# wenz116/lang2seg

Hardware: AMD Instinct MI355X
Metric: train images/sec (cycle loss on), 600×1000 input, at 1/2/4/8 MI355X (higher is better)
Workload: dtype bf16; 1 GPU; train_cycle.sh step: ResNet-101 C4 + 7 spatial dynamic filters + att2in2 cycle loss, 600x1000 image, 20-token expression (V=3349), 12000->2000 proposals, 256 RoIs, per-GPU batch 1; variant=cycle, parallelism=dp1

## Files before the change

include/lang2seg_hip.h:

```cpp
#ifndef LANG2SEG_HIP_H
#define LANG2SEG_HIP_H
#include <stdint.h>
#ifdef __HIPCC__
#include <hip/hip_runtime.h>
#else
typedef struct ihipStream_t* hipStream_t;
#endif
#ifdef __cplusplus
extern "C" {
#endif

#define L2S_F32 0
#define L2S_BF16 1

int l2s_version(void);

#define L2S_CONV_RELU 1
#define L2S_CONV_OUT_F32 4
#define L2S_CONV_DECONV2X2 8
#define L2S_CONV_SCATTER 16
#define L2S_ALGO_AUTO 0
#define L2S_ALGO_STAGED 1
#define L2S_ALGO_DMA 2
#define L2S_ALGO_DMA_STAMPED 4
// ... 5 lines not shown
#define L2S_ALGO_DMA256 9
#define L2S_ALGO_WS64_STAMPED 8
typedef struct {
  const void* x;
  const void* w;
  void* y;
  const float* bias;
  const void* add;
  const void* ref;
  int n_img, IH, IW, Cin, OH, OW, Cout, KH, KW, stride, pad;
  int ldx, ldy, ldadd, ldref;
  int flags;
  int out_h, out_w, out_stride;
  int tile;
  int split_k;
  int xcd_mode;
  int algo;
  float* ws;
  size_t ws_floats;
  int prio;
} l2s_conv_desc;
int l2s_conv_igemm(const l2s_conv_desc* d, int dtype, hipStream_t stream);
const char* l2s_conv_plan_name(const l2s_conv_desc* d, int dtype);
const char* l2s_last_kernel(void);

typedef struct {
  const void* dy;
  const void* x;
  float* dw;
  int n_img, IH, IW, Cin, OH, OW, Cout, KH, KW, stride, pad;
  int lddy, ldx;
  int split_k;
  int tile;
  float* ws;
  size_t ws_bytes;
} l2s_wgrad_desc;
size_t l2s_wgrad_ws_bytes(const l2s_wgrad_desc* d, int dtype);

#define L2S_WGRAD_MAX_GROUP 64
#define L2S_WGRAD_MAX_SEG 2
typedef struct {
  const void* dy[L2S_WGRAD_MAX_SEG];
  const void* x[L2S_WGRAD_MAX_SEG];
  int n_img[L2S_WGRAD_MAX_SEG], IH[L2S_WGRAD_MAX_SEG], IW[L2S_WGRAD_MAX_SEG], OH[L2S_WGRAD_MAX_SEG], OW[L2S_WGRAD_MAX_SEG];
  int lddy[L2S_WGRAD_MAX_SEG], ldx[L2S_WGRAD_MAX_SEG];
  float* dw;
// ... 370 lines not shown
```

lang2seg_amd/_lib.py:

```python
import ctypes as C
import os

_HERE = os.path.dirname(os.path.abspath(__file__))
LIB_PATH = os.path.join(_HERE, 'lib', 'liblang2seg_hip.so')
F32, BF16 = 0, 1

vp, i32, i64, f32, u64, sz = C.c_void_p, C.c_int, C.c_long, C.c_float, C.c_uint64, C.c_size_t


class ConvDesc(C.Structure):
    _fields_ = [('x', vp), ('w', vp), ('y', vp), ('bias', vp), ('add', vp), ('ref', vp),
                ('n_img', i32), ('IH', i32), ('IW', i32), ('Cin', i32), ('OH', i32), ('OW', i32), ('Cout', i32),
                ('KH', i32), ('KW', i32), ('stride', i32), ('pad', i32),
                ('ldx', i32), ('ldy', i32), ('ldadd', i32), ('ldref', i32), ('flags', i32),
                ('out_h', i32), ('out_w', i32), ('out_stride', i32), ('tile', i32), ('split_k', i32), ('xcd_mode', i32), ('algo', i32), ('ws', vp), ('ws_floats', sz), ('prio', i32)]


class RoiBlock0Desc(C.Structure):
    _fields_ = [('feat', vp), ('rois', vp), ('w1', vp), ('b1', vp), ('w2', vp), ('b2', vp), ('pooled', vp), ('y1', vp), ('y2', vp),
                ('H', i32), ('W', i32), ('C', i32), ('R', i32), ('P', i32), ('N1', i32), ('N2', i32), ('spatial_scale', C.c_float), ('debug', i32)]


class WgradDesc(C.Structure):
    _fields_ = [('dy', vp), ('x', vp), ('dw', vp),
# ... 84 lines not shown


class BeamStepArgs(C.Structure):
    _fields_ = [('logits', vp), ('ld_logits', i32)] + [(n, i32) for n in ('V1', 'B', 't', 'T', 'R', 'n_state')] + \
               [(n, vp) for n in ('beam_seq', 'beam_seq_logprobs', 'beam_logprobs_sum')] + \
               [('state_in', vp * 4), ('state_out', vp * 4), ('ld_in', i32 * 4), ('ld_out', i32 * 4)] + \
               [(n, vp) for n in ('next_tokens', 'parents', 'done', 'done_count')]


class SgdSeg(C.Structure):
    _fields_ = [('offset', i64), ('count', i64), ('row_len', i32), ('weight_decay', i32), ('rowscale_off', i64),
                ('lr_mult', f32), ('chunk0', i32), ('flags', i32), ('reserved', i32)]


CONV_RELU, CONV_OUT_F32, CONV_DECONV2X2, CONV_SCATTER = 1, 4, 8, 16
LOSS_RPN_CLS, LOSS_RPN_BOX, LOSS_CLS, LOSS_BOX, LOSS_MASK, LOSS_CAP, LOSS_TOTAL, LOSS_RESPONSE = range(8)

SIGS = {
    'l2s_version': (i32, []),
    'l2s_conv_plan_name': (C.c_char_p, [vp, i32]),
    'l2s_last_kernel': (C.c_char_p, []),
    'l2s_roialign_block0_fwd': (i32, [C.POINTER(RoiBlock0Desc), vp]),
    'l2s_conv_igemm': (i32, [C.POINTER(ConvDesc), i32, vp]),
    'l2s_conv_wgrad': (i32, [C.POINTER(WgradDesc), i32, vp]),
    'l2s_wgrad_ws_bytes': (sz, [C.POINTER(WgradDesc), i32]),
    'l2s_wgrad_variant': (i32, [i32, i32, i32, i32, i32, i32, i32, i64, i32]),
    'l2s_wgrad_tiles': (i64, [i32, i32, i32, i32, i32]),
    'l2s_conv_wgrad_grouped': (i32, [vp, vp, i32, i32, i32, vp, sz, vp]),
    'l2s_weight_cast': (i32, [vp, vp, vp, i32, i32, i32, i32, vp]),
    'l2s_weight_transpose': (i32, [vp, vp, vp, i32, i32, i32, i32, vp]),
    'l2s_colsum': (i32, [vp, i32, i32, i32, vp, vp, i64, i32, vp]),
    'l2s_weight_transpose_batched': (i32, [vp, i32, i32, i32, vp]),
    'l2s_stem_conv': (i32, [vp, vp, vp, vp, vp, i32, i32, i32, i32, i32, vp]),
    'l2s_stem_pack_bytes': (C.c_size_t, []),
    'l2s_stem_pack': (i32, [vp, vp, vp]),
    'l2s_stem_pool_bf16': (i32, [vp, vp, vp, vp, vp, i32, i32, i32, i32, i32, i32, vp]),
    'l2s_maxpool3x3s2': (i32, [vp, vp, i32, i32, i32, i32, i32, i32, vp]),
    'l2s_fill_f32': (i32, [vp, f32, i64, vp]),
    'l2s_cast': (i32, [vp, i32, vp, i32, i64, vp]),
    'l2s_add3': (i32, [vp, vp, vp, vp, i64, i32, vp]),
    'l2s_avgpool_fwd': (i32, [vp, vp, i32, i32, i32, i32, vp]),
    'l2s_avgpool_bwd': (i32, [vp, vp, vp, vp, i32, i32, i32, i32, vp]),
    'l2s_adaptive_pool_fwd': (i32, [vp, vp, vp, i32, i32, i32, i32, i32, i32, i32, vp]),
    'l2s_adaptive_pool_bwd': (i32, [vp, i32, i32, i32, vp, vp, vp, i32, i32, i32, i32, i32, i32, vp]),
    'l2s_mask_downsample': (i32, [vp, vp, i32, i32, i32, i32, vp]),
    'l2s_dropout_mask': (i32, [vp, i64, f32, vp, u64, vp]),
# ... 187 lines not shown
```

lang2seg_amd/csrc/conv_igemm.hip:

```cpp
#include "common.h"
#include "roi_sample.h"
#include "../../include/lang2seg_hip.h"
#include <stdlib.h>
#include <type_traits>

namespace {

template <typename T> struct Mma;
template <> struct Mma<bf16_t> {
  static __device__ __forceinline__ f32x4 run(const uint4& a, const uint4& b, f32x4 c) {
    return __builtin_amdgcn_mfma_f32_16x16x32_bf16(__builtin_bit_cast(bf16x8, a), __builtin_bit_cast(bf16x8, b), c, 0, 0, 0);
  }
};
template <> struct Mma<float> {
  static __device__ __forceinline__ f32x4 run(const uint4& a, const uint4& b, f32x4 c) {
    c = __builtin_amdgcn_mfma_f32_16x16x4f32(__uint_as_float(a.x), __uint_as_float(b.x), c, 0, 0, 0);
    c = __builtin_amdgcn_mfma_f32_16x16x4f32(__uint_as_float(a.y), __uint_as_float(b.y), c, 0, 0, 0);
    c = __builtin_amdgcn_mfma_f32_16x16x4f32(__uint_as_float(a.z), __uint_as_float(b.z), c, 0, 0, 0);
    c = __builtin_amdgcn_mfma_f32_16x16x4f32(__uint_as_float(a.w), __uint_as_float(b.w), c, 0, 0, 0);
    return c;
  }
};

constexpr int ROWB = 128;
// ... 1405 lines not shown
  const int rrow = lane >> 4, rch = lane & 15;
#pragma unroll
  for (int i = 0; i < TM; ++i) {
    if (i + 1 < TM) fetch(i + 1, ov[(i + 1) & 1]);
#pragma unroll
    for (int j = 0; j < TN; ++j) {
      const u32x2 oo = ov[i & 1][j];
      float v[4] = {acc[i][j][0] + bv[j][0], acc[i][j][1] + bv[j][1], acc[i][j][2] + bv[j][2], acc[i][j][3] + bv[j][3]};
      if constexpr (BOTH) igemm_finish<4, false>(p, v, oo, rv[i & 1][j]);
      else igemm_finish<4, false>(p, v, oo, oo);
      *(u32x2*)(wlds + fr * 256 + (((2 * j + (fg >> 1)) ^ fr) << 4) + ((fg & 1) << 3)) = igemm_pack_bf<u32x2>(v);
    }
#pragma unroll
    for (int h = 0; h < 4; ++h) {
      const int row = rrow + 4 * h;
      const u32x4v q = *(const u32x4v*)(wlds + row * 256 + ((rch ^ row) << 4));
      const int m = m0 + wm * WM + i * 16 + row, n = n0 + wn * WN + rch * 8;
      const unsigned o = (m < M && n < p.Cout) ? (unsigned)(((long)m * p.ldy + n) * 2) : NOPE;
      __builtin_amdgcn_raw_buffer_store_b128(q, ry, o, 0, 0);
    }
  }
}

__global__ __launch_bounds__(512) void igemm_dma256_kernel(const l2s_conv_desc p) {
  typedef bf16_t T;
  constexpr int BM = 256, BN = 256, WM = 64, WN = 128, TM = 4, TN = 8;
  constexpr int RB = 64;
  constexpr int STG = (BM + BN) * RB;
  constexpr int NP = 4;
  extern __shared__ __attribute__((aligned(16))) char smem[];
  const int tid = threadIdx.x, lane = tid & 63;
  const int wave = __builtin_amdgcn_readfirstlane(tid >> 6);
  const int grp = wave >> 2;
  const int wm = wave >> 1, wn = wave & 1;
  const int M = p.n_img * p.OH * p.OW;
  const int K = p.Cin;
  int mt, nt;
  igemm_tile_of(blockIdx.x, (M + BM - 1) / BM, (p.Cout + BN - 1) / BN, p.xcd_mode, mt, nt);
  const int m0 = mt * BM, n0 = nt * BN;
  const unsigned lds0 = (unsigned)(uintptr_t)(__attribute__((address_space(3))) char*)smem;
  i32x4s rx, rw;
  rx.x = (int)(uintptr_t)p.x; rx.y = (int)((uintptr_t)p.x >> 32); rx.z = (int)(((long)(M - 1) * p.ldx + p.Cin) * 2L); rx.w = 0x00020000;
  rw.x = (int)(uintptr_t)p.w; rw.y = (int)((uintptr_t)p.w >> 32); rw.z = (int)((long)p.Cout * K * 2L); rw.w = 0x00020000;
  const int prow = lane >> 2, sch = (lane & 3) ^ ((prow >> 2) & 3);
  unsigned voA[2], voB[2];
#pragma unroll
  for (int j = 0; j < 2; ++j) {
    const int m = m0 + 16 * (wave + 8 * j) + prow, n = n0 + 16 * (wave + 8 * j) + prow;
    voA[j] = m < M ? (unsigned)(((long)m * p.ldx + sch * 8) * 2L) : OOR;
    voB[j] = n < p.Cout ? (unsigned)(((long)n * K + sch * 8) * 2L) : OOR;
  }
  const int KT = K / 32;
  const unsigned ldsA = lds0 + (unsigned)(wave * 1024), ldsB = ldsA + (unsigned)(BM * RB);
  auto request = [&](int stage, int t) {
    const unsigned sb = (unsigned)(stage * STG), so = (unsigned)(t * RB);
#pragma unroll
    for (int j = 0; j < 2; ++j) dma_b128(rx, voA[j], so, ldsA + sb + (unsigned)(j * 8192));
#pragma unroll
    for (int j = 0; j < 2; ++j) dma_b128(rw, voB[j], so, ldsB + sb + (unsigned)(j * 8192));
  };
  f32x4 acc[TM][TN];
#pragma unroll
  for (int i = 0; i < TM; ++i)
#pragma unroll
    for (int j = 0; j < TN; ++j) acc[i][j] = (f32x4){0.f, 0.f, 0.f, 0.f};
  const int fr = lane & 15, fg = lane >> 4;
  const int ch = (fg ^ ((fr >> 2) & 3)) << 4;
  const int offa = (wm * WM + fr) * RB + ch, offb = BM * RB + (wn * WN + fr) * RB + ch;
  uint4 fa[TM], fb[TN];
  auto read_all = [&](int stage) {
    const char* base = smem + stage * STG;
#pragma unroll
    for (int i = 0; i < TM; ++i) fa[i] = *(const uint4*)(base + offa + i * 16 * RB);
#pragma unroll
    for (int j = 0; j < TN; ++j) fb[j] = *(const uint4*)(base + offb + j * 16 * RB);
  };
  auto mma_all = [&]() {
#pragma unroll
    for (int i = 0; i < TM; ++i)
#pragma unroll
      for (int j = 0; j < TN; ++j) acc[i][j] = Mma<T>::run(fb[j], fa[i], acc[i][j]);
  };
// ... 6 lines not shown
  for (int t = 0; t < KT; ++t) {
    const int st2 = st == 0 ? 2 : st - 1;
    read_all(st);
    if (t + 2 < KT) request(st2, t + 2);
    wait_lgkm0();
    if (grp == 1) {
      if (t + 2 < KT) asm volatile("s_waitcnt vmcnt(%0)" ::"n"(NP) : "memory");
      else asm volatile("s_waitcnt vmcnt(0)" ::: "memory");
    }
    wg_barrier();
    __builtin_amdgcn_sched_barrier(0);
    mma_all();
    __builtin_amdgcn_sched_barrier(0);
    if (grp == 0) {
      if (t + 2 < KT) asm volatile("s_waitcnt vmcnt(%0)" ::"n"(NP) : "memory");
      else asm volatile("s_waitcnt vmcnt(0)" ::: "memory");
    }
    wg_barrier();
    st = st == 2 ? 0 : st + 1;
  }
  if (grp == 0) wg_barrier();
  if (p.add && p.ref) igemm_epilogue_wave128<TM, TN, true>(p, acc, m0, n0, wm, wn, lane, M, smem + 3 * STG + wave * 4096);
  else igemm_epilogue_wave128<TM, TN, false>(p, acc, m0, n0, wm, wn, lane, M, smem + 3 * STG + wave * 4096);
}

template <int BM, int BN>
__global__ __launch_bounds__(512) void igemm_pdma_kernel(const l2s_conv_desc p) {
  typedef bf16_t T;
  constexpr int WGM = 4, WGN = 2, WM = BM / WGM, WN = BN / WGN, TM = WM / 16, TN = WN / 16;
  constexpr int PA = BM / 64, PB = BN / 64, NP = PA + PB;
  constexpr int STG = (BM + BN) * ROWB;
  extern __shared__ __attribute__((aligned(16))) char smem[];
  const int tid = threadIdx.x, lane = tid & 63;
  const int wave = __builtin_amdgcn_readfirstlane(tid >> 6);
  const int grp = wave >> 2;
  const int wm = wave >> 1, wn = wave & 1;
  const int M = p.n_img * p.OH * p.OW;
  const int K = p.Cin;
  const int KT = K / 64;
  const int MT = (M + BM - 1) / BM, NT = (p.Cout + BN - 1) / BN, G = MT * NT;
  const int ntl = (G - (int)blockIdx.x + (int)gridDim.x - 1) / (int)gridDim.x;
  auto tile_of = [&](int i, int& m0_, int& n0_) {
    int mt, nt;
    igemm_tile_of(blockIdx.x + i * gridDim.x, MT, NT, p.xcd_mode, mt, nt);
    m0_ = mt * BM; n0_ = nt * BN;
  };
// ... 622 lines not shown
int launch_igemm_p3(const l2s_conv_desc& d, hipStream_t st) {
  const int M = d.n_img * d.OH * d.OW;
  const size_t lds = (size_t)NS * 4 * ((PR / 16 + 9 * BN / 16 + 3) / 4) * 1024;
  IGEMM_LAUNCH_RETURN((igemm_p3_kernel<BN, PR, NS>), dim3(cdiv(M, 128) * cdiv(d.Cout, BN)), dim3(512), lds, st, d);
}

template <int BM, int BN, bool STAMP = false>
int launch_igemm_dma(const l2s_conv_desc& d, hipStream_t st) {
  const int M = d.n_img * d.OH * d.OW;
  const size_t lds = (size_t)3 * (BM + BN) * ROWB + (STAMP ? 8192 : 0);
  IGEMM_LAUNCH_RETURN((igemm_dma_kernel<BM, BN, STAMP>), dim3(cdiv(M, BM) * cdiv(d.Cout, BN)), dim3(512), lds, st, d);
}

int launch_igemm_dma196(const l2s_conv_desc& d, hipStream_t st) {
  const int M = d.n_img * d.OH * d.OW;
  const size_t lds = (size_t)3 * (256 + 128) * ROWB;
  IGEMM_LAUNCH_RETURN(igemm_dma196_kernel, dim3(cdiv(M, T196) * cdiv(d.Cout, 128)), dim3(512), lds, st, d);
}

int launch_igemm_dma256(const l2s_conv_desc& d, hipStream_t st) {
  const int M = d.n_img * d.OH * d.OW;
  const size_t lds = (size_t)3 * 512 * 64 + 8 * 4096;
  IGEMM_LAUNCH_RETURN(igemm_dma256_kernel, dim3(cdiv(M, 256) * cdiv(d.Cout, 256)), dim3(512), lds, st, d);
}

template <int BM, int BN>
int launch_igemm_pdma(const l2s_conv_desc& d, hipStream_t st) {
  const int M = d.n_img * d.OH * d.OW;
  const int G = cdiv(M, BM) * cdiv(d.Cout, BN);
  const int cap = l2s_knobs::pdma_wgs > 0 ? (l2s_knobs::pdma_wgs & ~7) : 256;
  const int grid = G < cap ? ((G + 7) & ~7) : cap;
  const size_t lds = (size_t)3 * (BM + BN) * ROWB + 8 * 2048;
  IGEMM_LAUNCH_RETURN((igemm_pdma_kernel<BM, BN>), dim3(grid), dim3(512), lds, st, d);
}
#undef IGEMM_LAUNCH_RETURN
#undef IGEMM_LAUNCH

}


enum ConvPlan { PLAN_EINVAL = 0, PLAN_GENERIC64, PLAN_GENERIC128, PLAN_RING64, PLAN_RING128, PLAN_WS64, PLAN_KS64, PLAN_KS64_D3, PLAN_SP224, PLAN_SP256,
                PLAN_DMA256, PLAN_DMA256_STAMPED, PLAN_WS64_SPLITK, PLAN_P3_32_256, PLAN_P3_64_256, PLAN_P3_32_384, PLAN_P3_64_384, PLAN_RING128X64, PLAN_PDMA256, PLAN_DMA256X256, PLAN_DMA196 };
static const char* const PLAN_NAMES[] = {"invalid", "igemm_kernel<64,64>", "igemm_kernel<128,128>", "igemm_ring_kernel<64,64>", "igemm_ring_kernel<128,128>",
                                         "igemm_ws64_kernel", "igemm_ks64_kernel<4>", "igemm_ks64_kernel<3>", "igemm_sp_kernel<224,128>", "igemm_sp_kernel<256,128>",
                                         "igemm_dma_kernel<256,128>", "igemm_dma_kernel<256,128,stamped>", "igemm_ws64_kernel + splitk_reduce_kernel", "igemm_p3_kernel<32,256>", "igemm_p3_kernel<64,256>", "igemm_p3_kernel<32,384>", "igemm_p3_kernel<64,384>", "igemm_ring_kernel<128,64>", "igemm_pdma_kernel<256,128>", "igemm_dma256_kernel", "igemm_dma196_kernel"};
static ConvPlan conv_plan(const l2s_conv_desc* d, int dtype, bool* tapin_out) {
// ... 89 lines not shown
    case PLAN_P3_64_256: return launch_igemm_p3<64, 256, 3>(dd, stream);
    case PLAN_P3_32_384: return launch_igemm_p3<32, 384, 3>(dd, stream);
    case PLAN_P3_64_384: return launch_igemm_p3<64, 384, 2>(dd, stream);
    case PLAN_KS64: return launch_igemm_ks64<4>(dd, stream);
    case PLAN_KS64_D3: return launch_igemm_ks64<3>(dd, stream);
    case PLAN_WS64:
      if (d->algo == L2S_ALGO_WS64_STAMPED) return launch_igemm_ws64<3, 64, true>(dd, stream);
      return launch_igemm_ws64<3, 64>(dd, stream);
    case PLAN_WS64_SPLITK: return launch_igemm_ws64<3, 64>(dd, stream, splitk_factor(dd, d->KH * d->KW * d->Cin / 64));
    case PLAN_SP224: return BYT(OUT_TAP(launch_igemm_sp, bf16_t, 224, 128, 2, 4, 2), OUT_TAP(launch_igemm_sp, float, 224, 128, 2, 4, 2));
    case PLAN_SP256: return BYT(OUT_TAP(launch_igemm_sp, bf16_t, 256, 128, 4, 2, 2), OUT_TAP(launch_igemm_sp, float, 256, 128, 4, 2, 2));
    case PLAN_RING128X64: return launch_igemm_ring<bf16_t, 128, 64, 2, 2, 2, false>(dd, stream);
    case PLAN_RING128: return BYT(OUT(launch_igemm_ring, bf16_t, 128, 128, 2, 2, 2), OUT(launch_igemm_ring, float, 128, 128, 2, 2, 2));
    case PLAN_RING64: return BYT(OUT(launch_igemm_ring, bf16_t, 64, 64, 2, 2, 2), OUT(launch_igemm_ring, float, 64, 64, 2, 2, 4));
    case PLAN_GENERIC128: return BYT(OUT(launch_igemm, bf16_t, 128, 128), OUT(launch_igemm, float, 128, 128));
    case PLAN_GENERIC64: return BYT(OUT(launch_igemm, bf16_t, 64, 64), OUT(launch_igemm, float, 64, 64));
    default: return L2S_EINVAL;
  }
#undef BYT
#undef OUT
#undef OUT_TAP
}

extern "C" int l2s_roialign_block0_fwd(const l2s_roi_block0_desc* d, hipStream_t stream) {
  if (!d || !d->feat || !d->rois || !d->w1 || !d->w2 || !d->pooled || !d->y1 || !d->y2) return L2S_EINVAL;
  const int PP = d->P * d->P;
  if (d->R <= 0 || PP < 1 || PP > 64 || d->C % 128 || d->N1 % 128 || d->N2 % 128 || d->N1 <= 0 || d->N2 <= 0) return L2S_EINVAL;
  if ((size_t)PP * d->C * 2 + 64 * sizeof(RoiTaps) > 160 * 1024) return L2S_EINVAL;
  if ((long)d->H * d->W * d->C * 2 >= (1L << 31) || (long)d->N1 * d->C * 2 >= (1L << 31) || (long)d->N2 * d->C * 2 >= (1L << 31)) return L2S_EINVAL;
  return launch_roialign_block0(*d, stream);
}
```

lang2seg_amd/nets/network.py:

```python
import numpy as np
import os
import torch

from .. import ops as O
from .._lib import F32, BF16, LOSS_CAP
from ..model.config import cfg
from .params import ParamStore
from . import anchors as ANC


class ConvOp(object):

    def __init__(self, net, wkey, Cin, Cout, k=1, stride=1, pad=0, bias_key=None, need_dgrad=True, group=None, Cout_pad=None, full_map=False):
        self.net, self.wkey, self.Cin, self.Cout, self.k, self.stride, self.pad = net, wkey, Cin, Cout, k, stride, pad
        self.full_map = bool(full_map and k > 1 and pad == 0 and stride == 1)
        self.t_taps, self.t_cin = (1, k * k * Cin) if self.full_map else (k * k, Cin)
        self.bias_key, self.need_dgrad, self.group = bias_key, need_dgrad, group
        self.Np = Cout if Cout_pad is None else Cout_pad
        self.prio = 1 if str(wkey).startswith(('resnet.layer1.', 'resnet.layer2.', 'resnet.layer3.')) and getattr(net, 'chain_prio', True) else 0
        P = net.P
        taps = k * k
        cnt = self.Np * taps * Cin
        if group is not None:
            self.trainable = True
# ... 11 lines not shown
            else:
                self.w_master = P.frozen[wkey].view(-1)
                self.w_grad = None
                self.wf = O.empty((cnt,), net.dt)
            if bias_key is not None and bias_key in P.offsets:
                self.bias = P.view(bias_key); self.bias_grad = P.view(bias_key, P.grad)
            elif bias_key is not None:
                self.bias = P.frozen[bias_key]; self.bias_grad = None
            else:
                self.bias = P.bn_bias.get(wkey); self.bias_grad = None
        self.wb = O.empty((cnt,), net.dt) if (need_dgrad and self.trainable) else None
        net.convs.append(self)

    def refresh(self, full=False):
        taps = self.k * self.k
        if not self.trainable and full:
            O.weight_cast(self.w_master, self.scale, self.wf, self.Np, taps, self.Cin)
        if self.wb is not None:
            O.weight_transpose(self.w_master, self.scale, self.wb, self.Np, self.t_taps, self.t_cin)

    def out_hw(self, IH, IW):
        return (IH + 2 * self.pad - self.k) // self.stride + 1, (IW + 2 * self.pad - self.k) // self.stride + 1

    def fwd(self, x, n, IH, IW, y, add=None, relu=False, out_f32=False, tile=0):
        OH, OW = self.out_hw(IH, IW)
        O.conv_igemm(x, self.wf, y, n, IH, IW, self.Cin, OH, OW, self.Np, self.k, self.k, self.stride, self.pad,
                     bias=self.bias, add=add, relu=relu, out_f32=out_f32, tile=tile, dt=self.net.dt, ws=self.net.splitk_ws(n * OH * OW * self.Np), prio=max(self.prio, self.net.prio_floor),
                     algo=(self.net.conv_algo if self.k == 1 and self.stride == 1 and self.Np >= 1024 else None))
        return y

    def dgrad(self, g, n, IH, IW, dx, add=None, ref=None):
        OH, OW = self.out_hw(IH, IW)
        if self.full_map:
            assert IH == self.k and IW == self.k and OH == 1 and OW == 1
            O.conv_igemm(g, self.wb, dx, n, 1, 1, self.Np, 1, 1, self.t_cin, 1, 1, 1, 0, add=add, ref=ref, dt=self.net.dt,
                         prio=max(self.prio, self.net.prio_floor))
            return dx
        if self.stride == 1:
            O.conv_igemm(g, self.wb, dx, n, OH, OW, self.Np, IH, IW, self.Cin, self.k, self.k, 1, self.k - 1 - self.pad,
                         add=add, ref=ref, dt=self.net.dt, ws=self.net.splitk_ws(n * IH * IW * self.Cin), prio=max(self.prio, self.net.prio_floor),
                         algo=(self.net.conv_algo if self.k == 1 and self.Cin >= 1024 else None))
        else:
            assert self.k == 1
            O.conv_igemm(g, self.wb, dx, n, OH, OW, self.Np, OH, OW, self.Cin, 1, 1, 1, 0, add=add, ref=ref,
                         scatter=(IH, IW, self.stride), dt=self.net.dt, prio=max(self.prio, self.net.prio_floor))
        return dx

    def wgrad(self, g, x, n, IH, IW):
        ko = self.net.knockout
        if 'wgrad' in ko or ('wgrad4' in ko and str(self.wkey).startswith('resnet.layer4.')) or \
                ('wgrad3' in ko and str(self.wkey).startswith(('resnet.layer3.', 'resnet.layer2.'))):
            return
        OH, OW = self.out_hw(IH, IW)
        self.net.wgq.add(self.w_grad, g, x, n, IH, IW, self.Cin, OH, OW, self.Np, self.k, self.stride, self.pad)
# ... 104 lines not shown
                        ctx.__enter__()
                    O.call('l2s_conv_wgrad_grouped', ent[1].data_ptr(), C.cast(arr, C.c_void_p), len(chunk), v, dt, ws.data_ptr(),
                           ws.numel() * 4, O.stream())
                    if ctx is not None:
                        ctx.__exit__(None, None, None)
        return True

    V5_STREAM = 'wg'
    SMALL_M_TILE = 0
    MIN_WG = 256
    V4_FILL = 128


class Bottleneck(object):

    def __init__(self, net, prefix, inplanes, planes, stride, has_down, need_dx=True):
        self.net, self.prefix, self.stride, self.need_dx = net, prefix, stride, need_dx
        self.inpl, self.planes = inplanes, planes
        self.c1 = ConvOp(net, prefix + '.conv1.weight', inplanes, planes, 1, stride, 0, need_dgrad=need_dx)
        self.c2 = ConvOp(net, prefix + '.conv2.weight', planes, planes, 3, 1, 1)
        self.c3 = ConvOp(net, prefix + '.conv3.weight', planes, planes * 4, 1, 1, 0)
        self.down = ConvOp(net, prefix + '.downsample.0.weight', inplanes, planes * 4, 1, stride, 0, need_dgrad=need_dx) if has_down else None

    def fwd(self, x, n, IH, IW, tag):
        net = self.net
        OH, OW = self.c1.out_hw(IH, IW)
        a1 = net.buf(tag + '.a1', (n * OH * OW, self.planes))
        a2 = net.buf(tag + '.a2', (n * OH * OW, self.planes))
        y = net.buf(tag + '.y', (n * OH * OW, self.planes * 4))
        self.c1.fwd(x, n, IH, IW, a1, relu=True)
        self.c2.fwd(a1, n, OH, OW, a2, relu=True)
        if self.down is not None:
            sc = net.buf(tag + '.sc', (n * OH * OW, self.planes * 4))
            self.down.fwd(x, n, IH, IW, sc)
            self.c3.fwd(a2, n, OH, OW, y, add=sc, relu=True)
        else:
            self.c3.fwd(a2, n, OH, OW, y, add=x, relu=True)
        return y, OH, OW, (x, a1, a2, IH, IW, OH, OW, n)

    def fwd_rest(self, x, a1, sc, n, IH, IW, tag):
        net = self.net
        a2 = net.buf(tag + '.a2', (n * IH * IW, self.planes))
        y = net.buf(tag + '.y', (n * IH * IW, self.planes * 4))
        self.c2.fwd(a1, n, IH, IW, a2, relu=True)
        self.c3.fwd(a2, n, IH, IW, y, add=sc, relu=True)
        return y, IH, IW, (x, a1, a2, IH, IW, IH, IW, n)

    def bwd(self, g, saved, tag, x_is_relu_out=True):
        net = self.net
        x, a1, a2, IH, IW, OH, OW, n = saved
        self.c3.wgrad(g, a2, n, OH, OW)
        dz2 = net.buf(tag + '.dz2', (n * OH * OW, self.planes))
        self.c3.dgrad(g, n, OH, OW, dz2, ref=a2)
        self.c2.wgrad(dz2, a1, n, OH, OW)
        dz1 = net.buf(tag + '.dz1', (n * OH * OW, self.planes))
        self.c2.dgrad(dz2, n, OH, OW, dz1, ref=a1)
        self.c1.wgrad(dz1, x, n, IH, IW)
        if self.down is not None:
            self.down.wgrad(g, x, n, IH, IW)
        if not self.need_dx:
            return None
        dx = net.buf(tag + '.dx', (n * IH * IW, self.inpl))
        ref = x if x_is_relu_out else None
        if self.down is not None:
            if self.stride != 1 and tag not in net._precleared:
                O.memset_zero(dx)
            self.c1.dgrad(dz1, n, IH, IW, dx)
            self.down.dgrad(g, n, IH, IW, dx, add=dx, ref=ref)
        else:
            self.c1.dgrad(dz1, n, IH, IW, dx, add=g, ref=ref)
        return dx


class Network(object):
    def __init__(self, batch_size=1):
        self._feat_stride = [16, ]
        self._batch_size = batch_size
        self._predictions = {}
        self._losses = {}
        self._anchor_targets = {}
        self._proposal_targets = {}
        self._mode = 'TRAIN'
        self.training = True
        self.device = 'cuda'
        self._bufs = {}
        self._buf_users = {}
        self.convs = []
# ... 293 lines not shown
            self._tr_tiles = sum(((c.Cin + 63) // 64) * ((c.Np + 63) // 64) * c.k * c.k for c in items)
        if self.use_streams and not full:
            S = self.streams()
            self.sfork(torch.cuda.current_stream(), S['tr'])
            with torch.cuda.stream(S['tr']):
                O.weight_transpose_batched(self._tr_table, self._tr_n, self._tr_tiles, self.dt)
            self._tr_pending = True
        else:
            O.weight_transpose_batched(self._tr_table, self._tr_n, self._tr_tiles, self.dt)

    update_on_wg = False
    defer_heads = False
    conv_algo = None
    roi_pdma = False
    layer1_fused = True
    cap_persistent = True
    _precleared = frozenset()
    prio_floor = 0
    cap_map_prio = 0
    rpn_wgrad_early = False
    rpn_bwd_early = True
    join_before_layer1 = False
    stem_mfma = True
    wgrad_overwrite = True
    update_clears_grad = False
    SLOT_UPDATE_REST = 0
    SLOT_UPDATE_L2 = 1
    SLOT_WGRADS = 2
    update_split = False
    layer2_side = False

    def join_update(self, full=True, layer2_only=False):
        if self.use_streams and self.update_on_wg:
            if layer2_only and self.update_split and not self.defer_heads and not getattr(self, '_pass_without_step', False):
                O.event_wait(self.SLOT_UPDATE_L2, torch.cuda.current_stream())
                if not self.layer2_side:
                    O.event_wait(self.SLOT_WGRADS, torch.cuda.current_stream())
            elif self.defer_heads and not full:
                O.event_wait(self.SLOT_UPDATE_REST, torch.cuda.current_stream())
            else:
                self.sfork(self.streams()['wg'], torch.cuda.current_stream())
                if self.layer2_side:
                    self.sfork(self.streams()['wg2'], torch.cuda.current_stream())

    def join_backlog(self):
        if self.use_streams and self.update_on_wg and self.layer2_side and self.update_split and not self.defer_heads \
# ... 106 lines not shown
```

lang2seg_amd/nets/resnet_v1.py:

```python
import os
import numpy as np
import torch

from .. import ops as O
from .._lib import F32, BF16
from ..model.config import cfg
from .network import Network, ConvOp, Bottleneck
from .params import ParamStore, encoder_config, caption_config
from .captioners import CAPTIONERS
from .variants import solver_cfg
from . import anchors as ANC
from . import decode
from . import caption_rows

f32 = torch.float32


class resnetv1(Network):
    variant = 'cycle'

    def __init__(self, opt, batch_size=1, num_layers=50, variant=None):
        Network.__init__(self, batch_size=batch_size)
        from .variants import VARIANTS
        if variant is not None:
# ... 389 lines not shown
    def _roi_trunk_fwd(self, net_conv, Hc, Wc, rois, n, saved=None):
        P, dt = self.P, self.dt
        C4, PS = self._C4_feat_dim, int(cfg.POOLING_SIZE)
        train = saved is not None
        tag = 'l4r' if train else 'l4t'
        saved = saved if train else {}
        blk0 = self.layers[4][0]
        kind, CS, mp = self._pool_mode()
        fused = (train and self.fuse_roialign and dt == BF16 and kind == 'crop' and not mp and blk0.down is not None and blk0.stride == 1 and
                 O.roialign_block0_ok(C4, PS, blk0.planes, blk0.planes * 4))
        if fused:
            pool5 = self.buf('roi.pool5', (n * PS * PS, C4))
            a1 = self.buf('l4r.0.a1', (n * PS * PS, blk0.planes)); sc = self.buf('l4r.0.sc', (n * PS * PS, blk0.planes * 4))
            O.roialign_block0_fwd(net_conv, Hc, Wc, C4, rois, n, PS, 1.0 / 16.0, blk0.c1.wf, blk0.c1.bias, blk0.planes,
                                  blk0.down.wf, blk0.down.bias, blk0.planes * 4, pool5, a1, sc)
            x, hh, ww, sv = blk0.fwd_rest(pool5, a1, sc, n, PS, PS, 'l4r.0')
            saved[('4r', 0)] = sv
        else:
            pool5 = self._rois_pool_fwd(net_conv, Hc, Wc, rois, n, saved)
            x, hh, ww = pool5, PS, PS
        for b, blk in enumerate(self.layers[4]):
            if fused and b == 0:
                continue
            x, hh, ww, sv = blk.fwd(x, n, hh, ww, '%s.%d' % (tag, b))
            saved[('4r', b)] = sv
        fc7s = x
        fc7 = self.buf('roi.fc7', (n, 2048))
        O.avgpool_fwd(fc7s, fc7, n, PS * PS, 2048)
        cheads = self.buf('roi.heads', (n, P.rcnn_npad), f32)
        self.rcnn_heads.fwd(fc7, n, 1, 1, cheads, out_f32=True)
        if train:
            self.t.update({'pool5': pool5, 'spatial_fc7': fc7s, 'rcnn_heads': cheads})
            saved['roi'] = (fc7s, fc7)
        return cheads, fc7s

    def _mask_fwd(self, fc7s, n):
        P = self.P
        PS, MS = int(cfg.POOLING_SIZE), int(cfg.MASK_SIZE)
        up = self.buf('mask.up', (n * MS * MS, 256))
        O.conv_igemm(fc7s, self.up_wT, up, n, PS, PS, 2048, PS, PS, 4 * 256, bias=P.view('mask_up_sampling.bias'), relu=True, deconv=True, dt=self.dt)
        mscore = self.buf('mask.score', (n * MS * MS, self._num_classes), f32)
        self.mask_pred.fwd(up, n, MS, MS, mscore, out_f32=True)
        return up, mscore

    def _roi_head_fwd(self, net_conv, Hc, Wc, rois, R, FGM, saved):
        cheads, fc7s = self._roi_trunk_fwd(net_conv, Hc, Wc, rois, R, saved)
        if fc7s is None:
# ... 524 lines not shown
```

lang2seg_amd/ops.py:

```python
import ctypes as C
import torch
from . import _lib
from ._lib import ptr, call, F32, BF16, ConvDesc, WgradDesc

TORCH_DT = {F32: torch.float32, BF16: torch.bfloat16}


def stream():
    return torch.cuda.current_stream().cuda_stream


def dt_of(t):
    return BF16 if t.dtype == torch.bfloat16 else F32


def empty(shape, dt, device='cuda'):
    return torch.empty(shape, dtype=TORCH_DT[dt], device=device)


def stream_fork(from_stream, to_stream):
    call('l2s_stream_fork', from_stream.cuda_stream, to_stream.cuda_stream)


def event_record(slot, s):
# ... 90 lines not shown
    if out_f32:
        fl |= _lib.CONV_OUT_F32
    if deconv:
        fl |= _lib.CONV_DECONV2X2
    if scatter is not None:
        fl |= _lib.CONV_SCATTER
        d.out_h, d.out_w, d.out_stride = scatter
    d.flags = fl
    d.tile = tile
    d.split_k = split_k
    d.xcd_mode = xcd_mode
    d.algo = CONV_ALGO if algo is None else algo
    d.ws = ptr(ws)
    d.ws_floats = 0 if ws is None else ws.numel()
    d.prio = prio
    global LAST_PLAN
    dtv = dt_of(x) if dt is None else dt
    if TRACK_PLAN:
        LAST_PLAN = _lib.load().l2s_conv_plan_name(C.byref(d), dtv).decode()
    call('l2s_conv_igemm', C.byref(d), dtv, stream())
    return y


def roialign_block0_fwd(feat, H, W, C_, rois, R, P, spatial_scale, w1, b1, N1, w2, b2, N2, pooled, y1, y2, debug=0):
    d = _lib.RoiBlock0Desc()
    d.feat, d.rois, d.w1, d.b1, d.w2, d.b2 = ptr(feat), ptr(rois), ptr(w1), ptr(b1), ptr(w2), ptr(b2)
    d.pooled, d.y1, d.y2 = ptr(pooled), ptr(y1), ptr(y2)
    d.H, d.W, d.C, d.R, d.P, d.N1, d.N2, d.spatial_scale = H, W, C_, R, P, N1, N2, float(spatial_scale)
    d.debug = debug
    call('l2s_roialign_block0_fwd', C.byref(d), stream())


def roialign_block0_ok(C_, P, N1, N2):
    return P * P <= 64 and C_ % 128 == 0 and N1 % 128 == 0 and N2 % 128 == 0 and P * P * C_ * 2 + 4096 <= 160 * 1024


def _wgrad_desc(dy, x, dw, n_img, IH, IW, Cin, OH, OW, Cout, KH, KW, stride, pad, lddy, ldx, split_k, tile, ws):
    d = WgradDesc()
    d.dy, d.x, d.dw = ptr(dy), ptr(x), ptr(dw)
    d.n_img, d.IH, d.IW, d.Cin, d.OH, d.OW, d.Cout = n_img, IH, IW, Cin, OH, OW, Cout
    d.KH, d.KW, d.stride, d.pad = KH, KW, stride, pad
    d.lddy = Cout if lddy is None else lddy
    d.ldx = Cin if ldx is None else ldx
    d.split_k, d.tile = split_k, tile
    d.ws = ptr(ws)
    d.ws_bytes = 0 if ws is None else ws.numel() * ws.element_size()
# ... 826 lines not shown
```

Measured before the change: 224.5 img/s.

## Fuse bottleneck entry conv1 and downsample 1x1 convs into paired igemm kernels

Adds a paired 256x256 DMA igemm kernel for the forward pass. It computes conv1 and the downsample projection, which share the same input, in one launch by splitting the N-tile range between the two convs. A second kernel does the dgrad by concatenating both convs' K loops into one accumulator, so the two input-gradient GEMMs and the separate accumulate/memset step become a single pass. Bottleneck entry blocks use it when the shapes qualify and fall back to the separate launches otherwise. This removes launches and extra writes and re-reads of dx, but requires stride-1 1x1 convs with Cout a multiple of 256 and M of at least 4096 rows (or tile==256).

```diff
diff --git a/include/lang2seg_hip.h b/include/lang2seg_hip.h
--- a/include/lang2seg_hip.h
+++ b/include/lang2seg_hip.h
@@ -51,6 +51,8 @@
 } l2s_conv_desc;
 int l2s_conv_igemm(const l2s_conv_desc* d, int dtype, hipStream_t stream);
 const char* l2s_conv_plan_name(const l2s_conv_desc* d, int dtype);
+int l2s_conv_pair_fwd(const l2s_conv_desc* d1, const l2s_conv_desc* d2, int dtype, hipStream_t stream);
+int l2s_conv_pair_dgrad(const l2s_conv_desc* d1, const l2s_conv_desc* d2, int dtype, hipStream_t stream);
 const char* l2s_last_kernel(void);
 
 typedef struct {
diff --git a/lang2seg_amd/_lib.py b/lang2seg_amd/_lib.py
--- a/lang2seg_amd/_lib.py
+++ b/lang2seg_amd/_lib.py
@@ -130,6 +130,8 @@
     'l2s_last_kernel': (C.c_char_p, []),
     'l2s_roialign_block0_fwd': (i32, [C.POINTER(RoiBlock0Desc), vp]),
     'l2s_conv_igemm': (i32, [C.POINTER(ConvDesc), i32, vp]),
+    'l2s_conv_pair_fwd': (i32, [C.POINTER(ConvDesc), C.POINTER(ConvDesc), i32, vp]),
+    'l2s_conv_pair_dgrad': (i32, [C.POINTER(ConvDesc), C.POINTER(ConvDesc), i32, vp]),
     'l2s_conv_wgrad': (i32, [C.POINTER(WgradDesc), i32, vp]),
     'l2s_wgrad_ws_bytes': (sz, [C.POINTER(WgradDesc), i32]),
     'l2s_wgrad_variant': (i32, [i32, i32, i32, i32, i32, i32, i32, i64, i32]),
diff --git a/lang2seg_amd/csrc/conv_igemm.hip b/lang2seg_amd/csrc/conv_igemm.hip
--- a/lang2seg_amd/csrc/conv_igemm.hip
+++ b/lang2seg_amd/csrc/conv_igemm.hip
@@ -1451,42 +1451,60 @@
   }
 }
 
-__global__ __launch_bounds__(512) void igemm_dma256_kernel(const l2s_conv_desc p) {
+template <bool KPAIR>
+__device__ __forceinline__ void igemm_dma256_tile(const l2s_conv_desc& p, const l2s_conv_desc& q, int mt, int nt, char* smem) {
   typedef bf16_t T;
   constexpr int BM = 256, BN = 256, WM = 64, WN = 128, TM = 4, TN = 8;
   constexpr int RB = 64;
   constexpr int STG = (BM + BN) * RB;
   constexpr int NP = 4;
-  extern __shared__ __attribute__((aligned(16))) char smem[];
   const int tid = threadIdx.x, lane = tid & 63;
   const int wave = __builtin_amdgcn_readfirstlane(tid >> 6);
   const int grp = wave >> 2;
   const int wm = wave >> 1, wn = wave & 1;
   const int M = p.n_img * p.OH * p.OW;
   const int K = p.Cin;
-  int mt, nt;
-  igemm_tile_of(blockIdx.x, (M + BM - 1) / BM, (p.Cout + BN - 1) / BN, p.xcd_mode, mt, nt);
   const int m0 = mt * BM, n0 = nt * BN;
   const unsigned lds0 = (unsigned)(uintptr_t)(__attribute__((address_space(3))) char*)smem;
-  i32x4s rx, rw;
+  i32x4s rx, rw, rx2, rw2;
   rx.x = (int)(uintptr_t)p.x; rx.y = (int)((uintptr_t)p.x >> 32); rx.z = (int)(((long)(M - 1) * p.ldx + p.Cin) * 2L); rx.w = 0x00020000;
   rw.x = (int)(uintptr_t)p.w; rw.y = (int)((uintptr_t)p.w >> 32); rw.z = (int)((long)p.Cout * K * 2L); rw.w = 0x00020000;
+  if constexpr (KPAIR) {
+    rx2.x = (int)(uintptr_t)q.x; rx2.y = (int)((uintptr_t)q.x >> 32); rx2.z = (int)(((long)(M - 1) * q.ldx + q.Cin) * 2L); rx2.w = 0x00020000;
+    rw2.x = (int)(uintptr_t)q.w; rw2.y = (int)((uintptr_t)q.w >> 32); rw2.z = (int)((long)p.Cout * q.Cin * 2L); rw2.w = 0x00020000;
+  }
   const int prow = lane >> 2, sch = (lane & 3) ^ ((prow >> 2) & 3);
-  unsigned voA[2], voB[2];
+  unsigned voA[2], voB[2], voA2[2], voB2[2];
 #pragma unroll
   for (int j = 0; j < 2; ++j) {
     const int m = m0 + 16 * (wave + 8 * j) + prow, n = n0 + 16 * (wave + 8 * j) + prow;
     voA[j] = m < M ? (unsigned)(((long)m * p.ldx + sch * 8) * 2L) : OOR;
     voB[j] = n < p.Cout ? (unsigned)(((long)n * K + sch * 8) * 2L) : OOR;
-  }
-  const int KT = K / 32;
+    if constexpr (KPAIR) {
+      voA2[j] = m < M ? (unsigned)(((long)m * q.ldx + sch * 8) * 2L) : OOR;
+      voB2[j] = n < p.Cout ? (unsigned)(((long)n * q.Cin + sch * 8) * 2L) : OOR;
+    }
+  }
+  const int KT1 = K / 32;
+  const int KT = KPAIR ? KT1 + q.Cin / 32 : KT1;
   const unsigned ldsA = lds0 + (unsigned)(wave * 1024), ldsB = ldsA + (unsigned)(BM * RB);
   auto request = [&](int stage, int t) {
-    const unsigned sb = (unsigned)(stage * STG), so = (unsigned)(t * RB);
-#pragma unroll
-    for (int j = 0; j < 2; ++j) dma_b128(rx, voA[j], so, ldsA + sb + (unsigned)(j * 8192));
-#pragma unroll
-    for (int j = 0; j < 2; ++j) dma_b128(rw, voB[j], so, ldsB + sb + (unsigned)(j * 8192));
+    const unsigned sb = (unsigned)(stage * STG);
+    if constexpr (KPAIR) {
+      const bool second = t >= KT1;
+      const i32x4s ra = second ? rx2 : rx, rb = second ? rw2 : rw;
+      const unsigned so = (unsigned)((second ? t - KT1 : t) * RB);
+#pragma unroll
+      for (int j = 0; j < 2; ++j) dma_b128(ra, second ? voA2[j] : voA[j], so, ldsA + sb + (unsigned)(j * 8192));
+#pragma unroll
+      for (int j = 0; j < 2; ++j) dma_b128(rb, second ? voB2[j] : voB[j], so, ldsB + sb + (unsigned)(j * 8192));
+    } else {
+      const unsigned so = (unsigned)(t * RB);
+#pragma unroll
+      for (int j = 0; j < 2; ++j) dma_b128(rx, voA[j], so, ldsA + sb + (unsigned)(j * 8192));
+#pragma unroll
+      for (int j = 0; j < 2; ++j) dma_b128(rw, voB[j], so, ldsB + sb + (unsigned)(j * 8192));
+    }
   };
   f32x4 acc[TM][TN];
 #pragma unroll
@@ -1539,6 +1557,31 @@
   if (grp == 0) wg_barrier();
   if (p.add && p.ref) igemm_epilogue_wave128<TM, TN, true>(p, acc, m0, n0, wm, wn, lane, M, smem + 3 * STG + wave * 4096);
   else igemm_epilogue_wave128<TM, TN, false>(p, acc, m0, n0, wm, wn, lane, M, smem + 3 * STG + wave * 4096);
+}
+
+__global__ __launch_bounds__(512) void igemm_dma256_kernel(const l2s_conv_desc p) {
+  extern __shared__ __attribute__((aligned(16))) char smem[];
+  int mt, nt;
+  igemm_tile_of(blockIdx.x, (p.n_img * p.OH * p.OW + 255) / 256, (p.Cout + 255) / 256, p.xcd_mode, mt, nt);
+  igemm_dma256_tile<false>(p, p, mt, nt, smem);
+}
+
+struct conv_pair_args { l2s_conv_desc d[2]; };
+
+__global__ __launch_bounds__(512) void igemm_pair256_fwd_kernel(const conv_pair_args a) {
+  extern __shared__ __attribute__((aligned(16))) char smem[];
+  const int NT1 = a.d[0].Cout / 256, NT = NT1 + a.d[1].Cout / 256;
+  int mt, nt;
+  igemm_tile_of(blockIdx.x, (a.d[0].n_img * a.d[0].OH * a.d[0].OW + 255) / 256, NT, a.d[0].xcd_mode, mt, nt);
+  const l2s_conv_desc& p = a.d[nt >= NT1];
+  igemm_dma256_tile<false>(p, p, mt, nt >= NT1 ? nt - NT1 : nt, smem);
+}
+
+__global__ __launch_bounds__(512) void igemm_pair256_dgrad_kernel(const conv_pair_args a) {
+  extern __shared__ __attribute__((aligned(16))) char smem[];
+  int mt, nt;
+  igemm_tile_of(blockIdx.x, (a.d[0].n_img * a.d[0].OH * a.d[0].OW + 255) / 256, a.d[0].Cout / 256, a.d[0].xcd_mode, mt, nt);
+  igemm_dma256_tile<true>(a.d[0], a.d[1], mt, nt, smem);
 }
 
 template <int BM, int BN>
@@ -2207,6 +2250,15 @@
   const int M = d.n_img * d.OH * d.OW;
   const size_t lds = (size_t)3 * 512 * 64 + 8 * 4096;
   IGEMM_LAUNCH_RETURN(igemm_dma256_kernel, dim3(cdiv(M, 256) * cdiv(d.Cout, 256)), dim3(512), lds, st, d);
+}
+
+int launch_igemm_pair256(const l2s_conv_desc& d1, const l2s_conv_desc& d2, bool dgrad, hipStream_t st) {
+  const int M = d1.n_img * d1.OH * d1.OW;
+  const size_t lds = (size_t)3 * 512 * 64 + 8 * 4096;
+  conv_pair_args a;
+  a.d[0] = d1; a.d[1] = d2;
+  if (dgrad) IGEMM_LAUNCH_RETURN(igemm_pair256_dgrad_kernel, dim3(cdiv(M, 256) * (d1.Cout / 256)), dim3(512), lds, st, a);
+  IGEMM_LAUNCH_RETURN(igemm_pair256_fwd_kernel, dim3(cdiv(M, 256) * ((d1.Cout + d2.Cout) / 256)), dim3(512), lds, st, a);
 }
 
 template <int BM, int BN>
@@ -2342,6 +2394,35 @@
 #undef OUT_TAP
 }
 
+static bool pair256_ok(const l2s_conv_desc& d) {
+  if (!d.x || !d.w || !d.y || d.KH != 1 || d.KW != 1 || d.stride != 1 || d.pad != 0 || d.IH != d.OH || d.IW != d.OW) return false;
+  if (d.flags & ~L2S_CONV_RELU) return false;
+  const long M = (long)d.n_img * d.OH * d.OW;
+  if (M <= 0 || M >= (1 << 24) || d.Cin <= 0 || d.Cin % 32 || d.ldx % 8 || d.Cout <= 0 || d.Cout % 256) return false;
+  if (M * d.ldx * 2 >= (1L << 31) || (long)d.Cout * d.Cin * 2 >= (1L << 31) || !igemm_rows31(d, M)) return false;
+  return !(d.ldy & 7) && !((uintptr_t)d.y & 15) && !(d.ldadd & 3) && !(d.ldref & 3);
+}
+static bool pair256_rows(const l2s_conv_desc& d) { return (long)d.n_img * d.OH * d.OW >= 4096 || d.tile == 256; }
+
+extern "C" int l2s_conv_pair_fwd(const l2s_conv_desc* d1, const l2s_conv_desc* d2, int dtype, hipStream_t stream) {
+  if (!d1 || !d2 || dtype != L2S_BF16 || !pair256_ok(*d1) || !pair256_ok(*d2) || !pair256_rows(*d1)) return L2S_EINVAL;
+  if (d1->x != d2->x || d1->ldx != d2->ldx || d1->Cin != d2->Cin || d1->n_img != d2->n_img || d1->OH != d2->OH || d1->OW != d2->OW) return L2S_EINVAL;
+  if (d1->add || d1->ref || d2->add || d2->ref) return L2S_EINVAL;
+  l2s_conv_desc a = *d1, b = *d2;
+  a.xcd_mode = b.xcd_mode = 0;
+  return launch_igemm_pair256(a, b, false, stream);
+}
+
+extern "C" int l2s_conv_pair_dgrad(const l2s_conv_desc* d1, const l2s_conv_desc* d2, int dtype, hipStream_t stream) {
+  if (!d1 || !d2 || dtype != L2S_BF16 || !pair256_ok(*d1) || !pair256_ok(*d2) || !pair256_rows(*d1)) return L2S_EINVAL;
+  if (d1->y != d2->y || d1->ldy != d2->ldy || d1->Cout != d2->Cout || d1->ref != d2->ref || d1->ldref != d2->ldref ||
+      d1->n_img != d2->n_img || d1->OH != d2->OH || d1->OW != d2->OW) return L2S_EINVAL;
+  if (d1->add || d2->add || d1->bias || d2->bias || d1->flags || d2->flags) return L2S_EINVAL;
+  l2s_conv_desc a = *d1, b = *d2;
+  a.xcd_mode = b.xcd_mode = 0;
+  return launch_igemm_pair256(a, b, true, stream);
+}
+
 extern "C" int l2s_roialign_block0_fwd(const l2s_roi_block0_desc* d, hipStream_t stream) {
   if (!d || !d->feat || !d->rois || !d->w1 || !d->w2 || !d->pooled || !d->y1 || !d->y2) return L2S_EINVAL;
   const int PP = d->P * d->P;
diff --git a/lang2seg_amd/nets/network.py b/lang2seg_amd/nets/network.py
--- a/lang2seg_amd/nets/network.py
+++ b/lang2seg_amd/nets/network.py
@@ -57,14 +57,28 @@
     def out_hw(self, IH, IW):
         return (IH + 2 * self.pad - self.k) // self.stride + 1, (IW + 2 * self.pad - self.k) // self.stride + 1
 
-    def fwd(self, x, n, IH, IW, y, add=None, relu=False, out_f32=False, tile=0):
+    def pairs_with(self, c1):
+        return (self.net.dt == BF16 and self.k == 1 and c1.k == 1 and self.stride == 1 and c1.stride == 1 and self.pad == 0 and c1.pad == 0 and
+                self.Cin == c1.Cin)
+
+    def fwd(self, x, n, IH, IW, y, add=None, relu=False, out_f32=False, tile=0, pair=None):
+        if pair is not None:
+            c1, y1 = pair
+            ok = add is None and not out_f32 and self.pairs_with(c1) and \
+                O.conv_pair_fwd(x, n, IH, IW, self.Cin, c1.wf, c1.bias, y1, c1.Np, True, self.wf, self.bias, y, self.Np, relu)
+            return y if ok else None
         OH, OW = self.out_hw(IH, IW)
         O.conv_igemm(x, self.wf, y, n, IH, IW, self.Cin, OH, OW, self.Np, self.k, self.k, self.stride, self.pad,
                      bias=self.bias, add=add, relu=relu, out_f32=out_f32, tile=tile, dt=self.net.dt, ws=self.net.splitk_ws(n * OH * OW * self.Np), prio=max(self.prio, self.net.prio_floor),
                      algo=(self.net.conv_algo if self.k == 1 and self.stride == 1 and self.Np >= 1024 else None))
         return y
 
-    def dgrad(self, g, n, IH, IW, dx, add=None, ref=None):
+    def dgrad(self, g, n, IH, IW, dx, add=None, ref=None, pair=None):
+        if pair is not None:
+            c1, dz1 = pair
+            ok = add is None and self.pairs_with(c1) and self.wb is not None and c1.wb is not None and \
+                O.conv_pair_dgrad(dz1, c1.wb, c1.Np, g, self.wb, self.Np, dx, n, IH, IW, self.Cin, ref=ref)
+            return dx if ok else None
         OH, OW = self.out_hw(IH, IW)
         if self.full_map:
             assert IH == self.k and IW == self.k and OH == 1 and OW == 1
@@ -215,17 +229,22 @@
         self.c3 = ConvOp(net, prefix + '.conv3.weight', planes, planes * 4, 1, 1, 0)
         self.down = ConvOp(net, prefix + '.downsample.0.weight', inplanes, planes * 4, 1, stride, 0, need_dgrad=need_dx) if has_down else None
 
-    def fwd(self, x, n, IH, IW, tag):
+    def fwd(self, x, n, IH, IW, tag, pair=True):
         net = self.net
         OH, OW = self.c1.out_hw(IH, IW)
         a1 = net.buf(tag + '.a1', (n * OH * OW, self.planes))
         a2 = net.buf(tag + '.a2', (n * OH * OW, self.planes))
         y = net.buf(tag + '.y', (n * OH * OW, self.planes * 4))
-        self.c1.fwd(x, n, IH, IW, a1, relu=True)
+        paired = False
+        if self.down is not None:
+            sc = net.buf(tag + '.sc', (n * OH * OW, self.planes * 4))
+            paired = pair and net.pair_entry and self.down.fwd(x, n, IH, IW, sc, pair=(self.c1, a1)) is not None
+        if not paired:
+            self.c1.fwd(x, n, IH, IW, a1, relu=True)
         self.c2.fwd(a1, n, OH, OW, a2, relu=True)
         if self.down is not None:
-            sc = net.buf(tag + '.sc', (n * OH * OW, self.planes * 4))
-            self.down.fwd(x, n, IH, IW, sc)
+            if not paired:
+                self.down.fwd(x, n, IH, IW, sc)
             self.c3.fwd(a2, n, OH, OW, y, add=sc, relu=True)
         else:
             self.c3.fwd(a2, n, OH, OW, y, add=x, relu=True)
@@ -256,6 +275,8 @@
         dx = net.buf(tag + '.dx', (n * IH * IW, self.inpl))
         ref = x if x_is_relu_out else None
         if self.down is not None:
+            if net.pair_entry and self.down.dgrad(g, n, IH, IW, dx, ref=ref, pair=(self.c1, dz1)) is not None:
+                return dx
             if self.stride != 1 and tag not in net._precleared:
                 O.memset_zero(dx)
             self.c1.dgrad(dz1, n, IH, IW, dx)
@@ -595,6 +616,7 @@
     rpn_bwd_early = True
     join_before_layer1 = False
     stem_mfma = True
+    pair_entry = True
     wgrad_overwrite = True
     update_clears_grad = False
     SLOT_UPDATE_REST = 0
diff --git a/lang2seg_amd/nets/resnet_v1.py b/lang2seg_amd/nets/resnet_v1.py
--- a/lang2seg_amd/nets/resnet_v1.py
+++ b/lang2seg_amd/nets/resnet_v1.py
@@ -435,7 +435,7 @@
         for b, blk in enumerate(self.layers[4]):
             if fused and b == 0:
                 continue
-            x, hh, ww, sv = blk.fwd(x, n, hh, ww, '%s.%d' % (tag, b))
+            x, hh, ww, sv = blk.fwd(x, n, hh, ww, '%s.%d' % (tag, b), pair=train)
             saved[('4r', b)] = sv
         fc7s = x
         fc7 = self.buf('roi.fc7', (n, 2048))
diff --git a/lang2seg_amd/ops.py b/lang2seg_amd/ops.py
--- a/lang2seg_amd/ops.py
+++ b/lang2seg_amd/ops.py
@@ -136,6 +136,47 @@
     return y
 
 
+PAIR_KERNELS = {'l2s_conv_pair_fwd': 'igemm_pair256_fwd_kernel', 'l2s_conv_pair_dgrad': 'igemm_pair256_dgrad_kernel'}
+
+
+def _pair_desc(x, w, y, n_img, H, W, Cin, Cout, bias=None, ref=None, relu=False, ldx=None, ldy=None, ldref=None, tile=0):
+    d = ConvDesc()
+    d.x, d.w, d.y, d.bias, d.ref = ptr(x), ptr(w), ptr(y), ptr(bias), ptr(ref)
+    d.n_img, d.IH, d.IW, d.Cin, d.OH, d.OW, d.Cout = n_img, H, W, Cin, H, W, Cout
+    d.KH, d.KW, d.stride, d.pad = 1, 1, 1, 0
+    d.ldx = Cin if ldx is None else ldx
+    d.ldy = Cout if ldy is None else ldy
+    d.ldadd = d.ldy
+    d.ldref = Cout if ldref is None else ldref
+    d.flags = _lib.CONV_RELU if relu else 0
+    d.tile, d.xcd_mode = tile, -1
+    return d
+
+
+def _pair_call(name, d1, d2):
+    global LAST_PLAN
+    r = getattr(_lib.load(), name)(C.byref(d1), C.byref(d2), BF16, stream())
+    if r > 1:
+        raise _lib.L2SError('%s returned error %d' % (name, r))
+    if r == 0 and TRACK_PLAN:
+        LAST_PLAN = PAIR_KERNELS[name]
+    return r == 0
+
+
+def conv_pair_fwd(x, n_img, H, W, Cin, w1, b1, y1, N1, relu1, w2, b2, y2, N2, relu2, ldx=None, ldy1=None, ldy2=None, tile=0):
+    if x.dtype != torch.bfloat16:
+        return False
+    return _pair_call('l2s_conv_pair_fwd', _pair_desc(x, w1, y1, n_img, H, W, Cin, N1, bias=b1, relu=relu1, ldx=ldx, ldy=ldy1, tile=tile),
+                      _pair_desc(x, w2, y2, n_img, H, W, Cin, N2, bias=b2, relu=relu2, ldx=ldx, ldy=ldy2))
+
+
+def conv_pair_dgrad(g1, w1t, K1, g2, w2t, K2, dx, n_img, H, W, N, ref=None, ldg1=None, ldg2=None, ldy=None, ldref=None, tile=0):
+    if g1.dtype != torch.bfloat16:
+        return False
+    return _pair_call('l2s_conv_pair_dgrad', _pair_desc(g1, w1t, dx, n_img, H, W, K1, N, ref=ref, ldx=ldg1, ldy=ldy, ldref=ldref, tile=tile),
+                      _pair_desc(g2, w2t, dx, n_img, H, W, K2, N, ref=ref, ldx=ldg2, ldy=ldy, ldref=ldref))
+
+
 def roialign_block0_fwd(feat, H, W, C_, rois, R, P, spatial_scale, w1, b1, N1, w2, b2, N2, pooled, y1, y2, debug=0):
     d = _lib.RoiBlock0Desc()
     d.feat, d.rois, d.w1, d.b1, d.w2, d.b2 = ptr(feat), ptr(rois), ptr(w1), ptr(b1), ptr(w2), ptr(b2)
```

Measured after the change: 227.4 img/s, median of 3. 1.3% higher.
